# victordeleau/MUI-DeepAutoEncoder

Measured on NVIDIA B200. Metric: train samples/s, higher is better.
Workload: dtype bf16

## Files before the change

### include/codae_b200.h

```cpp
#ifndef CODAE_B200_H
#define CODAE_B200_H

#include <stddef.h>
#include <stdint.h>

#ifdef __cplusplus
extern "C" {
#endif

#define CODAE_VERSION 100

typedef struct codae_ctx codae_ctx;

enum codae_status { CODAE_OK = 0, CODAE_EINVAL = -1, CODAE_EARCH = -2, CODAE_ECUDA = -3, CODAE_ENOMEM = -4 };
enum codae_dtype { CODAE_F32 = 0, CODAE_BF16 = 1, CODAE_F32X3 = 2 };
enum codae_act { CODAE_ACT_NONE = 0, CODAE_ACT_RELU = 1 };
enum codae_metric { CODAE_METRIC_SQERR = 0, CODAE_METRIC_COSINE = 1 };
enum codae_vartype { CODAE_VAR_REGRESSION = 0, CODAE_VAR_CLASSIFICATION = 1 };
enum codae_engine { CODAE_ENGINE_SIMT_F32 = 0, CODAE_ENGINE_TCGEN05_BF16 = 1, CODAE_ENGINE_TCGEN05_F32X3 = 2 };

int codae_version(void);
int codae_ctx_create(int device, codae_ctx** out);
int codae_ctx_destroy(codae_ctx* ctx);
const char* codae_last_error(const codae_ctx* ctx);
int codae_ctx_sm_count(const codae_ctx* ctx);
enum codae_option { CODAE_OPT_SPLITK = 0, CODAE_OPT_PDL = 1, CODAE_OPT_PERSISTENT = 2, CODAE_OPT_WEIGHT_PREFETCH = 3,
                    CODAE_OPT_TMA_STORE = 4, CODAE_OPT_TMA_STORE_PERSISTENT = 5, CODAE_OPT_CTA_PAIR = 6 };
int codae_ctx_set_option(codae_ctx* ctx, int option, int value);
int codae_weights_written(codae_ctx* ctx, void* stream);
int codae_ctx_get_option(const codae_ctx* ctx, int option);
int codae_linear_engine(const codae_ctx* ctx, int dtype, int M, int N, int K);

int codae_mask_table_philox(codae_ctx* ctx, uint64_t seed, int64_t first_obs, int64_t n_obs, int nb_run,
                            int16_t* out, void* stream);

int codae_corrupt_fwd(codae_ctx* ctx, const float* data, int64_t n_rows, int64_t ld_data, const int64_t* batch_idx, int B,
                      const int16_t* mask_table, int nb_run, int run, const uint64_t* mask_bits,
                      const uint8_t* col_var, int io, void* out_cx, int cx_dtype, int64_t ld_cx, float* out_x,
                      int64_t ld_x, int32_t* out_mask_id, void* stream);

int codae_dense_masks(codae_ctx* ctx, const int64_t* batch_idx, int B, const int16_t* mask_table, int nb_run,
                      int run, const uint64_t* mask_bits, const uint8_t* nb_missing, const uint8_t* col_var, int io,
// ... 16 lines not shown
                        const float* norm_scale, const float* norm_min, int norm_first, const int32_t* mask_id,
                        const uint64_t* mask_bits, const uint8_t* nb_missing, int k_max, float* out_loss, double* acc,
                        void* stream);

int codae_linear_fwd(codae_ctx* ctx, const void* X, int64_t ldx, const void* W, int64_t ldw, const float* bias,
                     void* Y, int64_t ldy, int M, int N, int K, int act, int dtype, int out_dtype, void* stream);
int codae_linear_dgrad(codae_ctx* ctx, const void* dY, int64_t lddy, const void* W, int64_t ldw, const void* A_prev,
                       int64_t lda, void* dX, int64_t lddx, int M, int N, int K, int dtype, int out_dtype,
                       void* stream);
int codae_linear_wgrad(codae_ctx* ctx, const void* dY, int64_t lddy, const void* X, int64_t ldx, float* dW,
                       int64_t lddw, float* db, int M, int N, int K, int dtype, void* stream);
int codae_linear_wgrad_sq_slots(const codae_ctx* ctx, int M, int N, int K, int dtype);
int codae_linear_wgrad_sq(codae_ctx* ctx, const void* dY, int64_t lddy, const void* X, int64_t ldx, float* dW,
                          int64_t lddw, int M, int N, int K, int dtype, double* sq_partials, int n_slots,
                          void* stream);
int codae_linear_fwd_x3(codae_ctx* ctx, const void* X, int64_t ldx, int64_t x_plane, const void* W, int64_t ldw, int64_t w_plane,
                        void* Y, int64_t ldy, int64_t y_plane, int M, int N, int K, int act, int out_dtype, void* stream);
int codae_linear_dgrad_x3(codae_ctx* ctx, const void* dY, int64_t lddy, int64_t dy_plane, const void* W, int64_t ldw,
                          int64_t w_plane, const void* A_prev_hi, int64_t lda, void* dX, int64_t lddx, int64_t dx_plane, int M,
                          int N, int K, int out_dtype, void* stream);
int codae_linear_wgrad_x3(codae_ctx* ctx, const void* dY, int64_t lddy, int64_t dy_plane, const void* X, int64_t ldx,
                          int64_t x_plane, float* dW, int64_t lddw, int M, int N, int K, double* sq_partials, int n_slots,
                          void* stream);
int codae_split_x3(codae_ctx* ctx, const float* src, void* dst, int64_t n, int64_t plane_stride, void* stream);
typedef struct codae_tiny_layer {
    int64_t w_off;
    int32_t ld, bcol, in, out, relu;
} codae_tiny_layer;
int codae_tiny_mlp_fwd(codae_ctx* ctx, const codae_tiny_layer* layers, int n_layers, const float* flat, float* const* acts,
                       int64_t ld_act, int B, void* stream);
// ... 94 lines not shown
```

### mui-deepautoencoder_b200/codae/_C.py

```python
import ctypes
import os
import threading

import torch

_HERE = os.path.dirname(os.path.abspath(__file__))
LIB_PATH = os.path.join(_HERE, "_lib", "libcodae_b200.so")

OK, EINVAL, EARCH, ECUDA, ENOMEM = 0, -1, -2, -3, -4
F32, BF16, F32X3 = 0, 1, 2
ACT_NONE, ACT_RELU = 0, 1
METRIC_SQERR, METRIC_COSINE = 0, 1
VAR_REGRESSION, VAR_CLASSIFICATION = 0, 1
ENGINE_SIMT_F32, ENGINE_TCGEN05_BF16, ENGINE_TCGEN05_F32X3 = 0, 1, 2

_c = ctypes
_vp, _i, _i64, _u64, _f, _d, _sz = _c.c_void_p, _c.c_int, _c.c_int64, _c.c_uint64, _c.c_float, _c.c_double, _c.c_size_t

SIGNATURES = {
    "codae_version": (_i, []),
    "codae_ctx_create": (_i, [_i, _c.POINTER(_vp)]),
    "codae_ctx_destroy": (_i, [_vp]),
    "codae_last_error": (_c.c_char_p, [_vp]),
    "codae_ctx_sm_count": (_i, [_vp]),
# ... 2 lines not shown
    "codae_weights_written": (_i, [_vp, _vp]),
    "codae_linear_engine": (_i, [_vp, _i, _i, _i, _i]),
    "codae_mask_table_philox": (_i, [_vp, _u64, _i64, _i64, _i, _vp, _vp]),
    "codae_corrupt_fwd": (_i, [_vp, _vp, _i64, _i64, _vp, _i, _vp, _i, _i, _vp, _vp, _i, _vp, _i, _i64, _vp, _i64, _vp, _vp]),
    "codae_dense_masks": (_i, [_vp, _vp, _i, _vp, _i, _i, _vp, _vp, _vp, _i, _i, _vp, _vp, _vp]),
    "codae_mul_mask": (_i, [_vp, _vp, _vp, _vp, _i64, _vp]),
    "codae_loss_workspace_bytes": (_sz, [_vp]),
    "codae_mse_loss_fwd_bwd": (_i, [_vp, _vp, _i64, _vp, _vp, _i, _i64, _vp, _vp, _vp, _i, _i, _f, _vp, _i, _i64, _vp, _vp, _sz, _vp]),
    "codae_mixed_loss_fwd_bwd": (_i, [_vp, _vp, _vp, _i, _i, _i64, _i, _vp, _vp, _vp, _vp, _vp, _vp, _vp]),
    "codae_mixed_monitor": (_i, [_vp, _vp, _vp, _i, _i, _i64, _i, _vp, _vp, _vp, _vp, _vp, _i, _vp, _vp, _vp, _i, _vp, _vp, _vp]),
    "codae_linear_fwd": (_i, [_vp, _vp, _i64, _vp, _i64, _vp, _vp, _i64, _i, _i, _i, _i, _i, _i, _vp]),
    "codae_linear_dgrad": (_i, [_vp, _vp, _i64, _vp, _i64, _vp, _i64, _vp, _i64, _i, _i, _i, _i, _i, _vp]),
    "codae_linear_wgrad": (_i, [_vp, _vp, _i64, _vp, _i64, _vp, _i64, _vp, _i, _i, _i, _i, _vp]),
    "codae_linear_wgrad_sq_slots": (_i, [_vp, _i, _i, _i, _i]),
    "codae_linear_wgrad_sq": (_i, [_vp, _vp, _i64, _vp, _i64, _vp, _i64, _i, _i, _i, _i, _vp, _i, _vp]),
    "codae_linear_fwd_x3": (_i, [_vp, _vp, _i64, _i64, _vp, _i64, _i64, _vp, _i64, _i64, _i, _i, _i, _i, _i, _vp]),
    "codae_linear_dgrad_x3": (_i, [_vp, _vp, _i64, _i64, _vp, _i64, _i64, _vp, _i64, _vp, _i64, _i64, _i, _i, _i, _i, _vp]),
    "codae_linear_wgrad_x3": (_i, [_vp, _vp, _i64, _i64, _vp, _i64, _i64, _vp, _i64, _i, _i, _i, _vp, _i, _vp]),
    "codae_split_x3": (_i, [_vp, _vp, _vp, _i64, _i64, _vp]),
    "codae_tiny_mlp_fwd": (_i, [_vp, _vp, _i, _vp, _vp, _i64, _i, _vp]),
    "codae_tiny_mlp_bwd": (_i, [_vp, _vp, _i, _vp, _vp, _vp, _i64, _vp, _i64, _i, _vp]),
    "codae_cast_bf16": (_i, [_vp, _vp, _vp, _i64, _vp]),
    "codae_sqnorm_workspace_bytes": (_sz, [_vp]),
    "codae_grad_sqnorm": (_i, [_vp, _vp, _i64, _vp, _vp, _sz, _vp]),
    "codae_adam_step": (_i, [_vp, _vp, _vp, _vp, _vp, _vp, _i, _i64, _d, _d, _d, _d, _d, _i, _d, _vp, _d, _vp, _vp]),
    "codae_clip_adam_step": (_i, [_vp, _vp, _vp, _vp, _vp, _vp, _i, _i64, _d, _d, _d, _d, _d, _i, _d, _vp, _vp, _sz, _d, _vp, _vp]),
    "codae_adam_step_partials": (_i, [_vp, _vp, _vp, _vp, _vp, _vp, _i, _i64, _d, _d, _d, _d, _d, _i, _d, _vp, _i, _vp, _d, _vp, _vp]),
    "codae_counter_add": (_i, [_vp, _vp, _i, _vp]),
    "codae_dp_workspace_bytes": (_sz, [_vp]),
    "codae_dp_shard_elems": (_i64, [_i64, _i]),
# ... 74 lines not shown
    c = _ctxs.get(dev)
    if c is None:
        with _lock:
            c = _ctxs.get(dev)
            if c is None:
                out = _vp()
                rc = lib().codae_ctx_create(dev, ctypes.byref(out))
                if rc != OK:
                    raise RuntimeError("codae_ctx_create failed (%d): %s" % (rc, (lib().codae_last_error(None) or b"").decode()))
                c = out
                _ctxs[dev] = c
    return c


OPT_SPLITK, OPT_PDL, OPT_PERSISTENT, OPT_WEIGHT_PREFETCH, OPT_TMA_STORE, OPT_TMA_STORE_PERSISTENT, OPT_CTA_PAIR = 0, 1, 2, 3, 4, 5, 6


def set_option(device, option, value):
    c = ctx(device)
    check(lib().codae_ctx_set_option(c, option, 1 if value else 0), c)


def weights_written(device):
    c = ctx(device)
    check(lib().codae_weights_written(c, stream()), c)


def get_option(device, option):
    v = lib().codae_ctx_get_option(ctx(device), option)
    if v < 0:
# ... 147 lines not shown
def linear_wgrad(dY, X, dW, db, M, N, K, dtype):
    c = ctx(dY.device)
    if dtype == F32X3:
        assert is_x3(dY) and is_x3(X) and db is None, "codae: the fp32-parity engine takes the bias gradient from the augmented column"
        check(lib().codae_linear_wgrad_x3(c, p(dY), ld(dY), dY.stride(0), p(X), ld(X), X.stride(0), p(dW), dW.stride(0), M, N, K,
                                          None, 0, stream()), c)
        return
    check(lib().codae_linear_wgrad(c, p(dY), dY.stride(0), p(X), X.stride(0), p(dW), dW.stride(0), p(db), M, N, K, dtype,
                                   stream()), c)


def linear_wgrad_sq_slots(device, M, N, K, dtype):
    return int(lib().codae_linear_wgrad_sq_slots(ctx(device), M, N, K, dtype))


def linear_wgrad_sq(dY, X, dW, M, N, K, dtype, sq_partials):
    c = ctx(dY.device)
    if dtype == F32X3:
        assert is_x3(dY) and is_x3(X)
        check(lib().codae_linear_wgrad_x3(c, p(dY), ld(dY), dY.stride(0), p(X), ld(X), X.stride(0), p(dW), dW.stride(0), M, N, K,
                                          p(sq_partials), sq_partials.numel(), stream()), c)
        return
    check(lib().codae_linear_wgrad_sq(c, p(dY), dY.stride(0), p(X), X.stride(0), p(dW), dW.stride(0), M, N, K, dtype,
                                      p(sq_partials), sq_partials.numel(), stream()), c)


def split_x3(src, dst):
    assert dst.dtype == torch.bfloat16 and dst.shape[0] == 3 and src.dtype == torch.float32
    assert src.is_contiguous() and dst[0].is_contiguous() and dst[0].numel() == src.numel()
    c = ctx(src.device)
    check(lib().codae_split_x3(c, p(src), p(dst), src.numel(), dst.stride(0), stream()), c)
# ... 232 lines not shown
```

### mui-deepautoencoder_b200/codae/tool/fused_step.py

```python
import os

import torch

from codae import _C
from codae.tool.metering import arch_tables


def _round_up(x, m):
    return (x + m - 1) // m * m


class FusedStep:

    BUCKET_BYTES = 32 << 20

    def __init__(self, model, corrupter, data, lr, weight_decay, clip=True, betas=(0.9, 0.999), eps=1e-8,
                 max_norm=1.0, world_size=1, process_group=None, use_graph=False, mixed=None, overlap_allreduce=True,
                 fused_clip_adam=True, wgrad_sqnorm=None, tiny_mlp=None, dp_mode=None):
        if model.flat is None:
            raise RuntimeError("codae: FusedStep needs model.to(cuda_device) first; there is no CPU fallback")
        if not data.is_cuda:
            raise RuntimeError("codae: FusedStep needs dataset.to(cuda_device) first; there is no CPU fallback")
        self.model, self.corrupter, self.data = model, corrupter, data
        self.lr, self.wd, self.clip, self.betas, self.eps, self.max_norm = lr, weight_decay, clip, betas, eps, max_norm
        self.world_size, self.pg = world_size, process_group
        self.use_graph = use_graph
        self.mixed = mixed
        self.overlap_allreduce = overlap_allreduce
        self.fused_clip_adam = fused_clip_adam
# ... 139 lines not shown
        if self.adt == "x3":
            return _C.new_x3((B, w), self.dev)
        return torch.zeros((B, w), dtype=self.adt, device=self.dev)

    def _buffers(self, B):
        b = self._bufs.get(B)
        if b is None:
            dev, adt, dims = self.dev, self.adt, self.model.dims
            M = self.model
            wmax = max(M.act_width(max(i, o)) for i, o in dims)
            width = (lambda w: wmax) if self.mixed is not None else (lambda w: None)
            acts = [M.new_activation(B, dims[0][0], adt, dev, width(dims[0][0]))]
            for l, (i, o) in enumerate(dims):
                last = l == len(dims) - 1
                acts.append(M.new_activation(B, o, torch.float32 if last else adt, dev, width(o)))
            b = dict(acts=acts,
                     g0=self._new_grad(B, wmax), g1=self._new_grad(B, wmax), g2=self._new_grad(B, wmax),
                     mask_id=torch.zeros(B, dtype=torch.int32, device=dev),
                     idx=torch.zeros(B, dtype=torch.int64, device=dev),
                     x=torch.zeros((B, wmax), dtype=torch.float32, device=dev) if self.mixed is not None else None,
                     mon=torch.zeros((B, len(self.mixed["arch"])), dtype=torch.float32, device=dev) if self.mixed is not None else None)
            if self.wgrad_sqnorm:
                slots = [_C.linear_wgrad_sq_slots(dev, B, o, _round_up(i, 8) + 1, self.eng) for i, o in dims]
                if min(slots) < 1:
                    raise RuntimeError("codae: wgrad_sqnorm: the tensor-core engine cannot tile every layer of this model")
                offs = [0]
                for c in slots:
                    offs.append(offs[-1] + c)
                b["sq_off"] = offs
                b["sq_partials"] = torch.zeros(offs[-1], dtype=torch.float64, device=dev)
            self._bufs[B] = b
        return b

    def _enqueue(self, B, b, run, global_batch, data, idx, table, train=True):
        model, dims, eng = self.model, self.model.dims, self.eng
        L = len(dims)
        _, bits, col_var, nmiss = self.corrupter.device_tables()
        acts = b["acts"]
        n = 0
        _C.corrupt_fwd(data, idx, B, table, run, bits, col_var, self.io, acts[0], b["x"], b["mask_id"]); n += 1
        wflat = model.gemm_weights(eng)
        tiny = self.tiny_mlp and len({a.stride(0) for a in acts}) == 1
        if tiny:
            _C.tiny_mlp_fwd(self._tiny_layers, model.flat, acts, B); n += 1
        else:
            for l, (i, o) in enumerate(dims):
                _C.linear_fwd(acts[l], model.aug_view(wflat, l), None, acts[l + 1], B, o, _round_up(i, 8) + 1,
                              _C.ACT_RELU if model.relu[l] else _C.ACT_NONE, eng); n += 1
        y = acts[L]
        o_last = dims[L - 1][1]
        gbuf = [b["g0"], b["g1"], b["g2"]]
        g = gbuf[(L - 1) % 3][..., :_round_up(o_last, 8)]
        if self.mixed is None:
            _C.mse_loss_fwd_bwd(data, idx, y, b["mask_id"], bits, col_var, B, self.io, 2.0 / (global_batch * self.io),
                                g if train else None, self.acc, self.loss_ws); n += 1
        else:
            pos, size, typ = self.var_tables
            _C.mixed_loss_fwd_bwd(b["x"], y, pos, size, typ, self.weight, g, self.mixed_loss); n += 1
            _C.mixed_monitor(b["x"], y, pos, size, typ, self.norm_scale, self.norm_min, self.norm_first, b["mask_id"], bits,
                             nmiss, self.corrupter.k_max, b["mon"], self.mixed_acc); n += 1
        if not train:
            return n
        if tiny:
            _C.tiny_mlp_bwd(self._tiny_layers, model.flat, self.gflat, acts, gbuf, B); n += 1
            return n + self._enqueue_update(b.get("sq_partials"))
        overlap_comm = self.world_size > 1 and self.overlap_allreduce and self.dp_mode == "nccl"
        if overlap_comm:
            import torch.distributed as dist
        main = torch.cuda.current_stream()
        side = self._wgrad_stream if (self.tc and B <= 1024) else main
        wdone = [None] * L
        bucket_hi = None
        for l in range(L - 1, -1, -1):
            i, o = dims[l]
            gl = gbuf[l % 3][..., :_round_up(o, 8)]
            if side is not main:
                ready = torch.cuda.Event()
                ready.record(main)
                side.wait_event(ready)
            with torch.cuda.stream(side):
                if self.wgrad_sqnorm:
                    sq = b["sq_partials"][b["sq_off"][l]:b["sq_off"][l + 1]]
                    _C.linear_wgrad_sq(gl, acts[l], model.aug_view(self.gflat, l), B, o, _round_up(i, 8) + 1, eng, sq)
                else:
                    _C.linear_wgrad(gl, acts[l], model.aug_view(self.gflat, l), None, B, o, _round_up(i, 8) + 1, eng)
                n += 1
                wdone[l] = torch.cuda.Event()
                wdone[l].record(side)
            if overlap_comm:
                lo = self._layer_span[l][0]
                if bucket_hi is None:
                    bucket_hi = self._layer_span[l][1]
                if (bucket_hi - lo) * 4 >= self.BUCKET_BYTES or l == 0:
                    comm = self._comm_stream
                    comm.wait_event(wdone[l])
                    with torch.cuda.stream(comm):
                        dist.all_reduce(self.gflat[lo:bucket_hi], op=dist.ReduceOp.SUM, group=self.pg)
                    bucket_hi = None
            if l > 0:
                if l + 2 <= L - 1 and side is not main:
                    main.wait_event(wdone[l + 2])
                gp = gbuf[(l - 1) % 3][..., :_round_up(i, 8)]
                _C.linear_dgrad(gl, model.weight_view(wflat, l), acts[l] if model.relu[l - 1] else None, gp, B, o, i, eng); n += 1
        if side is not main:
            main.wait_stream(side)
        if overlap_comm:
            main.wait_stream(self._comm_stream)
        elif self.world_size > 1 and self.dp_mode == "nccl":
            import torch.distributed as dist
            dist.all_reduce(self.gflat, op=dist.ReduceOp.SUM, group=self.pg)
        return n + self._enqueue_update(b.get("sq_partials"))

    def _enqueue_update(self, sq_partials=None):
        model, eng = self.model, self.eng
        n = 0
        _C.counter_add(self.step_dev, 1); n += 1
        pb = model.gemm_weights(eng) if self.tc else None
# ... 183 lines not shown
```

### mui-deepautoencoder_b200/csrc/common.cuh

```cuda
#pragma once
#include <cuda_runtime.h>
#include <cuda_bf16.h>
#include <stdint.h>
#include <stdio.h>
#include <string.h>
#include <mutex>

#include "../../include/codae_b200.h"

struct CUtensorMap_st;

struct codae_ctx {
    int device;
    int sm_count;
    int cc_major, cc_minor;
    char err[512];
    void* encode_tiled;
    int splitk;
    int persistent;
    int pdl;
    int weight_prefetch;
    int tma_store;
    int tma_store_persistent;
    int cta_pair;
    int weights_dirty;
    cudaStream_t dirty_stream;
    std::mutex mu;
};

extern char g_codae_last_error[512];

int codae_fail(codae_ctx* ctx, int code, const char* fmt, ...);
int codae_check_launch(codae_ctx* ctx, const char* what);

#define CODAE_REQUIRE(ctx, cond, ...)                                     \
    do {                                                                  \
        if (!(cond)) return codae_fail((ctx), CODAE_EINVAL, __VA_ARGS__); \
    } while (0)

// ... 129 lines not shown
```

### mui-deepautoencoder_b200/csrc/ctx.cu

```cuda
#include <stdarg.h>
#include <stdlib.h>

#include "common.cuh"

char g_codae_last_error[512] = "";

int codae_fail(codae_ctx* ctx, int code, const char* fmt, ...) {
    char buf[512];
    va_list ap;
    va_start(ap, fmt);
    vsnprintf(buf, sizeof(buf), fmt, ap);
    va_end(ap);
    if (ctx) {
        std::lock_guard<std::mutex> lk(ctx->mu);
        snprintf(ctx->err, sizeof(ctx->err), "%s", buf);
    }
    snprintf(g_codae_last_error, sizeof(g_codae_last_error), "%s", buf);
    return code;
}

int codae_check_launch(codae_ctx* ctx, const char* what) {
    cudaError_t e = cudaPeekAtLastError();
    if (e != cudaSuccess) {
        cudaGetLastError();
// ... 48 lines not shown
    c->pdl = 1;
    c->persistent = 1;
    c->weight_prefetch = 1;
    {
        const char* e = getenv("CODAE_TMA_STORE");
        c->tma_store = e ? (atoi(e) != 0) : 1;
    }
    {
        const char* e = getenv("CODAE_TMA_STORE_PERSISTENT");
        c->tma_store_persistent = e ? (atoi(e) != 0) : 1;
    }
    {
        const char* e = getenv("CODAE_CTA_PAIR");
        c->cta_pair = e ? (atoi(e) != 0) : 1;
    }
    c->weights_dirty = 0;
    c->dirty_stream = nullptr;
    void* fn = nullptr;
    cudaDriverEntryPointQueryResult qres;
    e = cudaGetDriverEntryPoint("cuTensorMapEncodeTiled", &fn, cudaEnableDefault, &qres);
    if (e == cudaSuccess && qres == cudaDriverEntryPointSuccess) c->encode_tiled = fn;
    else cudaGetLastError();
    *out = c;
    return CODAE_OK;
}

int codae_ctx_destroy(codae_ctx* ctx) {
    delete ctx;
    return CODAE_OK;
}

const char* codae_last_error(const codae_ctx* ctx) { return ctx ? ctx->err : g_codae_last_error; }

int codae_ctx_sm_count(const codae_ctx* ctx) { return ctx ? ctx->sm_count : 0; }

int codae_ctx_set_option(codae_ctx* ctx, int option, int value) {
    if (!ctx) return codae_fail(nullptr, CODAE_EINVAL, "codae_ctx_set_option: ctx is NULL");
    if (option == CODAE_OPT_SPLITK) ctx->splitk = value ? 1 : 0;
    else if (option == CODAE_OPT_PDL) ctx->pdl = value ? 1 : 0;
    else if (option == CODAE_OPT_PERSISTENT) ctx->persistent = value ? 1 : 0;
    else if (option == CODAE_OPT_WEIGHT_PREFETCH) ctx->weight_prefetch = value ? 1 : 0;
    else if (option == CODAE_OPT_TMA_STORE) ctx->tma_store = value ? 1 : 0;
    else if (option == CODAE_OPT_TMA_STORE_PERSISTENT) ctx->tma_store_persistent = value ? 1 : 0;
    else if (option == CODAE_OPT_CTA_PAIR) ctx->cta_pair = value ? 1 : 0;
    else return codae_fail(ctx, CODAE_EINVAL, "codae_ctx_set_option: unknown option %d", option);
    return CODAE_OK;
}

int codae_weights_written(codae_ctx* ctx, void* stream) {
    if (!ctx) return codae_fail(nullptr, CODAE_EINVAL, "codae_weights_written: ctx is NULL");
    codae_mark_weights_written(ctx, as_stream(stream));
    return CODAE_OK;
}

int codae_ctx_get_option(const codae_ctx* ctx, int option) {
    if (!ctx) return CODAE_EINVAL;
    switch (option) {
        case CODAE_OPT_SPLITK: return ctx->splitk;
        case CODAE_OPT_PDL: return ctx->pdl;
        case CODAE_OPT_PERSISTENT: return ctx->persistent;
        case CODAE_OPT_WEIGHT_PREFETCH: return ctx->weight_prefetch;
        case CODAE_OPT_TMA_STORE: return ctx->tma_store;
        case CODAE_OPT_TMA_STORE_PERSISTENT: return ctx->tma_store_persistent;
        case CODAE_OPT_CTA_PAIR: return ctx->cta_pair;
        default: return CODAE_EINVAL;
    }
}

}
```

### mui-deepautoencoder_b200/csrc/gemm.h

```cpp
#pragma once
#include <cuda.h>

#include "common.cuh"

int codae_simt_linear_fwd(codae_ctx* ctx, const float* X, int64_t ldx, const float* W, int64_t ldw, const float* bias,
                          float* Y, int64_t ldy, int M, int N, int K, int act, cudaStream_t s);
int codae_simt_linear_dgrad(codae_ctx* ctx, const float* dY, int64_t lddy, const float* W, int64_t ldw, const float* A_prev,
                            int64_t lda, float* dX, int64_t lddx, int M, int N, int K, cudaStream_t s);
int codae_simt_linear_wgrad(codae_ctx* ctx, const float* dY, int64_t lddy, const float* X, int64_t ldx, float* dW,
                            int64_t lddw, int M, int N, int K, cudaStream_t s);
int codae_colsum(codae_ctx* ctx, const void* dY, int dtype, int64_t ld, int M, int N, float* db, cudaStream_t s);

struct Tc05Gemm {
    const void* A; int64_t lda; bool a_kmajor;
    const void* B; int64_t ldb; bool b_kmajor;
    void* C; int64_t ldc; int c_dtype;
    int M, N, K;
    const float* bias; int act;
    const void* mask_src; int64_t ldm;
    bool b_is_weight = false;
    double* sq_partial = nullptr;
    int sq_slots = 0;
    int planes = 1;
    int64_t a_plane_stride = 0, b_plane_stride = 0, c_plane_stride = 0;
};
bool codae_tc05_supported(const codae_ctx* ctx, const Tc05Gemm& g);
int codae_tc05_gemm(codae_ctx* ctx, const Tc05Gemm& g, cudaStream_t s);
int codae_tc05_gemm_ctas(const codae_ctx* ctx, const Tc05Gemm& g);
int codae_tc05_make_map(codae_ctx* ctx, CUtensorMap* map, const void* base, long long rows, long long cols, long long ld,
                        int box_cols, int box_rows, int planes, long long plane_stride);

struct ScoreTcPass {
    int metric;
    const void* cat; int cat_planes;
    int64_t cat_ld, cat_plane_stride;
    int64_t n_rows, row0;
    const __nv_bfloat16* q_planes;
    int64_t q_ld, q_plane_stride;
    int Q, E, qb0, G, W, kp;
    const float* cc;
    const float* qq;
    float inv_scale, c_rel;
    float* ls; int64_t* li;
// ... 5 lines not shown
```

### mui-deepautoencoder_b200/csrc/gemm_tcgen05.cu

```cuda
#include <cuda.h>
#include <stdlib.h>

#include "common.cuh"
#include "gemm.h"
#include "tc05_ptx.cuh"

namespace {

constexpr int kThreads = 192;
constexpr int kMaxSplit = 8;
inline int x3_chunk_kb() {
    static const int v = [] {
        const char* e = getenv("CODAE_X3_CHUNK_KB");
        const int x = e ? atoi(e) : 0;
        return x >= 1 && x <= 64 ? x : 8;
    }();
    return v;
}
constexpr uint32_t kPersistentStageBytes = 4 * 2 * 4096;

struct Params {
    int M, N, K;
    int a_kmajor, b_kmajor;
    void* C;
// ... 773 lines not shown
            if (lane == 0) asm volatile("cp.async.bulk.wait_group.read 0;" ::: "memory");
            __syncwarp();
        }
        if (p.sq_partial) sq_partial_store(p.sq_partial + blockIdx.x, sq_acc, sq_red);
    }
    tc_fence_before();
    if constexpr (kPair) cluster_sync();
    else __syncthreads();
    if (warp == 1) {
        tc_fence_after();
        if constexpr (kPair) tmem_dealloc_pair(tmem_base, 2 * BN);
        else tmem_dealloc(tmem_base, 2 * BN);
    }
}


int g_trace_cta = 0;
unsigned long long* g_trace_buf = nullptr;

typedef CUresult (*EncodeTiledFn)(CUtensorMap*, CUtensorMapDataType, cuuint32_t, void*, const cuuint64_t*, const cuuint64_t*,
                                  const cuuint32_t*, const cuuint32_t*, CUtensorMapInterleave, CUtensorMapSwizzle,
                                  CUtensorMapL2promotion, CUtensorMapFloatOOBfill);

int make_map(codae_ctx* ctx, CUtensorMap* map, const void* base, long long rows, long long cols, long long ld, int box_cols,
             int box_rows, int planes = 1, long long plane_stride = 0) {
    const cuuint64_t dims[3] = {(cuuint64_t)cols, (cuuint64_t)rows, (cuuint64_t)planes};
    const cuuint64_t strides[2] = {(cuuint64_t)ld * 2, (cuuint64_t)plane_stride * 2};
    const cuuint32_t box[3] = {(cuuint32_t)box_cols, (cuuint32_t)box_rows, 1};
    const cuuint32_t estr[3] = {1, 1, 1};
    CUresult r = reinterpret_cast<EncodeTiledFn>(ctx->encode_tiled)(
// ... 340 lines not shown
        case 256: return launch<256>(ctx, g, s);
        case 128: return launch<128>(ctx, g, s);
        default: return launch<64>(ctx, g, s);
    }
}

int codae_tc05_gemm_ctas(const codae_ctx* ctx, const Tc05Gemm& g) {
    if (!ctx || !ctx->encode_tiled || g.M < 1 || g.N < 32 || g.K < 1) return 0;
    if (g.planes == 3) return pick_bn(ctx, g) == 128 ? make_plan<128, 3>(ctx, g).ctas : make_plan<64, 3>(ctx, g).ctas;
    switch (pick_bn(ctx, g)) {
        case 256: return make_plan<256>(ctx, g).ctas;
        case 128: return make_plan<128>(ctx, g).ctas;
        default: return make_plan<64>(ctx, g).ctas;
    }
}
```

### mui-deepautoencoder_b200/csrc/linear.cu

```cuda
#include "common.cuh"
#include "gemm.h"

namespace {
inline bool tc_shape_ok(int M, int N, int K) { return M >= 1 && N >= 32 && K >= 32; }
}

extern "C" {

int codae_linear_engine(const codae_ctx* ctx, int dtype, int M, int N, int K) {
    if (!ctx) return CODAE_EINVAL;
    if (dtype == CODAE_BF16 && ctx->encode_tiled && tc_shape_ok(M, N, K))
        return CODAE_ENGINE_TCGEN05_BF16;
    if (dtype == CODAE_F32X3 && ctx->encode_tiled && tc_shape_ok(M, N, K)) return CODAE_ENGINE_TCGEN05_F32X3;
    return CODAE_ENGINE_SIMT_F32;
}

int codae_linear_fwd(codae_ctx* ctx, const void* X, int64_t ldx, const void* W, int64_t ldw, const float* bias, void* Y,
                     int64_t ldy, int M, int N, int K, int act, int dtype, int out_dtype, void* stream) {
    CODAE_REQUIRE(ctx, ctx && X && W && Y, "codae_linear_fwd: NULL argument");
    CODAE_REQUIRE(ctx, M >= 1 && N >= 1 && K >= 1 && ldx >= K && ldw >= K && ldy >= N, "codae_linear_fwd: bad shape M=%d N=%d K=%d", M, N, K);
    CODAE_REQUIRE(ctx, act == CODAE_ACT_NONE || act == CODAE_ACT_RELU, "codae_linear_fwd: bad activation %d", act);
    if (dtype == CODAE_F32) {
        CODAE_REQUIRE(ctx, out_dtype == CODAE_F32, "codae_linear_fwd: f32 engine writes f32");
        return codae_simt_linear_fwd(ctx, (const float*)X, ldx, (const float*)W, ldw, bias, (float*)Y, ldy, M, N, K, act, as_stream(stream));
// ... 41 lines not shown
    return codae_tc05_gemm_ctas(ctx, g);
}

int codae_linear_wgrad_sq(codae_ctx* ctx, const void* dY, int64_t lddy, const void* X, int64_t ldx, float* dW, int64_t lddw,
                          int M, int N, int K, int dtype, double* sq_partials, int n_slots, void* stream) {
    CODAE_REQUIRE(ctx, ctx && dY && X && dW && sq_partials, "codae_linear_wgrad_sq: NULL argument");
    CODAE_REQUIRE(ctx, M >= 1 && N >= 1 && K >= 1 && lddy >= N && ldx >= K && lddw >= K, "codae_linear_wgrad_sq: bad shape M=%d N=%d K=%d", M, N, K);
    CODAE_REQUIRE(ctx, dtype == CODAE_BF16, "codae_linear_wgrad_sq: tensor-core engine only (dtype %d)", dtype);
    CODAE_REQUIRE(ctx, (reinterpret_cast<uintptr_t>(sq_partials) & 7) == 0, "codae_linear_wgrad_sq: sq_partials must be 8-byte aligned");
    Tc05Gemm g{dY, lddy, false, X, ldx, false, dW, lddw, CODAE_F32, N, K, M, nullptr, CODAE_ACT_NONE, nullptr, 0};
    g.sq_partial = sq_partials;
    g.sq_slots = n_slots;
    return codae_tc05_gemm(ctx, g, as_stream(stream));
}

int codae_linear_fwd_x3(codae_ctx* ctx, const void* X, int64_t ldx, int64_t x_plane, const void* W, int64_t ldw, int64_t w_plane,
                        void* Y, int64_t ldy, int64_t y_plane, int M, int N, int K, int act, int out_dtype, void* stream) {
    CODAE_REQUIRE(ctx, ctx && X && W && Y, "codae_linear_fwd_x3: NULL argument");
    CODAE_REQUIRE(ctx, M >= 1 && N >= 1 && K >= 1 && ldx >= K && ldw >= K && ldy >= N, "codae_linear_fwd_x3: bad shape M=%d N=%d K=%d", M, N, K);
    CODAE_REQUIRE(ctx, act == CODAE_ACT_NONE || act == CODAE_ACT_RELU, "codae_linear_fwd_x3: bad activation %d", act);
    CODAE_REQUIRE(ctx, out_dtype == CODAE_F32 || out_dtype == CODAE_F32X3, "codae_linear_fwd_x3: output is f32 or its bf16 triple");
    Tc05Gemm g{X, ldx, true, W, ldw, true, Y, ldy, out_dtype, M, N, K, nullptr, act, nullptr, 0, true};
    g.planes = 3; g.a_plane_stride = x_plane; g.b_plane_stride = w_plane; g.c_plane_stride = y_plane;
    return codae_tc05_gemm(ctx, g, as_stream(stream));
}

int codae_linear_dgrad_x3(codae_ctx* ctx, const void* dY, int64_t lddy, int64_t dy_plane, const void* W, int64_t ldw,
                          int64_t w_plane, const void* A_prev_hi, int64_t lda, void* dX, int64_t lddx, int64_t dx_plane, int M,
                          int N, int K, int out_dtype, void* stream) {
    CODAE_REQUIRE(ctx, ctx && dY && W && dX, "codae_linear_dgrad_x3: NULL argument");
// ... 22 lines not shown
```

Measured before the change: 1.244 million.

## Batch all layers' weight-gradient GEMMs into one grouped persistent tcgen05 launch

Adds a grouped persistent CTA-pair kernel that computes the weight gradients of every layer in a single launch, using a segment table to map tile items to problems. The backward pass first runs every dgrad, then issues this one grouped wgrad call instead of interleaving per-layer wgrad launches on a side stream. The aim is to cut launch overhead and fill the tail of small per-layer GEMMs by load-balancing tiles across all SMs. In exchange, wgrad can no longer overlap with dgrad, one gradient buffer per layer is needed instead of three, and the path only applies to large bf16 batches when sqnorm or peer mode is enabled.

After: 1.275 million (median of 6 runs). 2.5% higher.

```diff
diff --git a/include/codae_b200.h b/include/codae_b200.h
--- a/include/codae_b200.h
+++ b/include/codae_b200.h
@@ -25,7 +25,8 @@
 const char* codae_last_error(const codae_ctx* ctx);
 int codae_ctx_sm_count(const codae_ctx* ctx);
 enum codae_option { CODAE_OPT_SPLITK = 0, CODAE_OPT_PDL = 1, CODAE_OPT_PERSISTENT = 2, CODAE_OPT_WEIGHT_PREFETCH = 3,
-                    CODAE_OPT_TMA_STORE = 4, CODAE_OPT_TMA_STORE_PERSISTENT = 5, CODAE_OPT_CTA_PAIR = 6 };
+                    CODAE_OPT_TMA_STORE = 4, CODAE_OPT_TMA_STORE_PERSISTENT = 5, CODAE_OPT_CTA_PAIR = 6,
+                    CODAE_OPT_GROUPED_WGRAD = 7 };
 int codae_ctx_set_option(codae_ctx* ctx, int option, int value);
 int codae_weights_written(codae_ctx* ctx, void* stream);
 int codae_ctx_get_option(const codae_ctx* ctx, int option);
@@ -72,6 +73,10 @@
 int codae_linear_wgrad_sq(codae_ctx* ctx, const void* dY, int64_t lddy, const void* X, int64_t ldx, float* dW,
                           int64_t lddw, int M, int N, int K, int dtype, double* sq_partials, int n_slots,
                           void* stream);
+int codae_linear_wgrad_sq_grouped_slots(const codae_ctx* ctx, int n, const int* M, const int* N, const int* K, int dtype);
+int codae_linear_wgrad_sq_grouped(codae_ctx* ctx, int n, const void* const* dY, const int64_t* lddy, const void* const* X,
+                                  const int64_t* ldx, float* const* dW, const int64_t* lddw, const int* M, const int* N,
+                                  const int* K, int dtype, double* sq_partials, int n_slots, void* stream);
 int codae_linear_fwd_x3(codae_ctx* ctx, const void* X, int64_t ldx, int64_t x_plane, const void* W, int64_t ldw, int64_t w_plane,
                         void* Y, int64_t ldy, int64_t y_plane, int M, int N, int K, int act, int out_dtype, void* stream);
 int codae_linear_dgrad_x3(codae_ctx* ctx, const void* dY, int64_t lddy, int64_t dy_plane, const void* W, int64_t ldw,
diff --git a/mui-deepautoencoder_b200/codae/_C.py b/mui-deepautoencoder_b200/codae/_C.py
--- a/mui-deepautoencoder_b200/codae/_C.py
+++ b/mui-deepautoencoder_b200/codae/_C.py
@@ -40,6 +40,8 @@
     "codae_linear_wgrad": (_i, [_vp, _vp, _i64, _vp, _i64, _vp, _i64, _vp, _i, _i, _i, _i, _vp]),
     "codae_linear_wgrad_sq_slots": (_i, [_vp, _i, _i, _i, _i]),
     "codae_linear_wgrad_sq": (_i, [_vp, _vp, _i64, _vp, _i64, _vp, _i64, _i, _i, _i, _i, _vp, _i, _vp]),
+    "codae_linear_wgrad_sq_grouped_slots": (_i, [_vp, _i, _vp, _vp, _vp, _i]),
+    "codae_linear_wgrad_sq_grouped": (_i, [_vp, _i, _vp, _vp, _vp, _vp, _vp, _vp, _vp, _vp, _vp, _i, _vp, _i, _vp]),
     "codae_linear_fwd_x3": (_i, [_vp, _vp, _i64, _i64, _vp, _i64, _i64, _vp, _i64, _i64, _i, _i, _i, _i, _i, _vp]),
     "codae_linear_dgrad_x3": (_i, [_vp, _vp, _i64, _i64, _vp, _i64, _i64, _vp, _i64, _vp, _i64, _i64, _i, _i, _i, _i, _vp]),
     "codae_linear_wgrad_x3": (_i, [_vp, _vp, _i64, _i64, _vp, _i64, _i64, _vp, _i64, _i, _i, _i, _vp, _i, _vp]),
@@ -144,6 +146,7 @@
 
 
 OPT_SPLITK, OPT_PDL, OPT_PERSISTENT, OPT_WEIGHT_PREFETCH, OPT_TMA_STORE, OPT_TMA_STORE_PERSISTENT, OPT_CTA_PAIR = 0, 1, 2, 3, 4, 5, 6
+OPT_GROUPED_WGRAD = 7
 
 
 def set_option(device, option, value):
@@ -321,7 +324,26 @@
     return int(lib().codae_linear_wgrad_sq_slots(ctx(device), M, N, K, dtype))
 
 
+def _arr(ctype, vals):
+    return (ctype * len(vals))(*vals)
+
+
+def linear_wgrad_sq_grouped_slots(device, M, N, K, dtype):
+    n = len(M)
+    return int(lib().codae_linear_wgrad_sq_grouped_slots(ctx(device), n, _arr(_i, M), _arr(_i, N), _arr(_i, K), dtype))
+
+
 def linear_wgrad_sq(dY, X, dW, M, N, K, dtype, sq_partials):
+    if isinstance(dY, (list, tuple)):
+        c = ctx(dY[0].device)
+        n = len(dY)
+        assert len(X) == len(dW) == len(M) == len(N) == len(K) == n
+        check(lib().codae_linear_wgrad_sq_grouped(c, n, _arr(_vp, [t.data_ptr() for t in dY]), _arr(_i64, [t.stride(0) for t in dY]),
+                                                  _arr(_vp, [t.data_ptr() for t in X]), _arr(_i64, [t.stride(0) for t in X]),
+                                                  _arr(_vp, [t.data_ptr() for t in dW]), _arr(_i64, [t.stride(0) for t in dW]),
+                                                  _arr(_i, M), _arr(_i, N), _arr(_i, K), dtype, p(sq_partials),
+                                                  0 if sq_partials is None else sq_partials.numel(), stream()), c)
+        return
     c = ctx(dY.device)
     if dtype == F32X3:
         assert is_x3(dY) and is_x3(X)
diff --git a/mui-deepautoencoder_b200/codae/tool/fused_step.py b/mui-deepautoencoder_b200/codae/tool/fused_step.py
--- a/mui-deepautoencoder_b200/codae/tool/fused_step.py
+++ b/mui-deepautoencoder_b200/codae/tool/fused_step.py
@@ -13,6 +13,7 @@
 class FusedStep:
 
     BUCKET_BYTES = 32 << 20
+    SMALL_BATCH = 1024
 
     def __init__(self, model, corrupter, data, lr, weight_decay, clip=True, betas=(0.9, 0.999), eps=1e-8,
                  max_norm=1.0, world_size=1, process_group=None, use_graph=False, mixed=None, overlap_allreduce=True,
@@ -182,13 +183,15 @@
             for l, (i, o) in enumerate(dims):
                 last = l == len(dims) - 1
                 acts.append(M.new_activation(B, o, torch.float32 if last else adt, dev, width(o)))
-            b = dict(acts=acts,
-                     g0=self._new_grad(B, wmax), g1=self._new_grad(B, wmax), g2=self._new_grad(B, wmax),
+            grouped = self._grouped_wgrad_slots(B)
+            b = dict(acts=acts, gbuf=[self._new_grad(B, wmax) for _ in range(len(dims) if grouped else 3)], grouped=grouped > 0,
                      mask_id=torch.zeros(B, dtype=torch.int32, device=dev),
                      idx=torch.zeros(B, dtype=torch.int64, device=dev),
                      x=torch.zeros((B, wmax), dtype=torch.float32, device=dev) if self.mixed is not None else None,
                      mon=torch.zeros((B, len(self.mixed["arch"])), dtype=torch.float32, device=dev) if self.mixed is not None else None)
-            if self.wgrad_sqnorm:
+            if self.wgrad_sqnorm and grouped:
+                b["sq_partials"] = torch.zeros(grouped, dtype=torch.float64, device=dev)
+            elif self.wgrad_sqnorm:
                 slots = [_C.linear_wgrad_sq_slots(dev, B, o, _round_up(i, 8) + 1, self.eng) for i, o in dims]
                 if min(slots) < 1:
                     raise RuntimeError("codae: wgrad_sqnorm: the tensor-core engine cannot tile every layer of this model")
@@ -199,6 +202,13 @@
                 b["sq_partials"] = torch.zeros(offs[-1], dtype=torch.float64, device=dev)
             self._bufs[B] = b
         return b
+
+    def _grouped_wgrad_slots(self, B):
+        if self.eng != _C.BF16 or B <= self.SMALL_BATCH or not (self.wgrad_sqnorm or self.dp_mode == "peer"):
+            return 0
+        dims = self.model.dims
+        return _C.linear_wgrad_sq_grouped_slots(self.dev, [B] * len(dims), [o for _, o in dims],
+                                                [_round_up(i, 8) + 1 for i, _ in dims], self.eng)
 
     def _enqueue(self, B, b, run, global_batch, data, idx, table, train=True):
         model, dims, eng = self.model, self.model.dims, self.eng
@@ -217,8 +227,8 @@
                               _C.ACT_RELU if model.relu[l] else _C.ACT_NONE, eng); n += 1
         y = acts[L]
         o_last = dims[L - 1][1]
-        gbuf = [b["g0"], b["g1"], b["g2"]]
-        g = gbuf[(L - 1) % 3][..., :_round_up(o_last, 8)]
+        gbuf = b["gbuf"]
+        g = gbuf[(L - 1) % len(gbuf)][..., :_round_up(o_last, 8)]
         if self.mixed is None:
             _C.mse_loss_fwd_bwd(data, idx, y, b["mask_id"], bits, col_var, B, self.io, 2.0 / (global_batch * self.io),
                                 g if train else None, self.acc, self.loss_ws); n += 1
@@ -232,16 +242,25 @@
         if tiny:
             _C.tiny_mlp_bwd(self._tiny_layers, model.flat, self.gflat, acts, gbuf, B); n += 1
             return n + self._enqueue_update(b.get("sq_partials"))
+        if b["grouped"]:
+            for l in range(L - 1, 0, -1):
+                i, o = dims[l]
+                _C.linear_dgrad(gbuf[l][..., :_round_up(o, 8)], model.weight_view(wflat, l), acts[l] if model.relu[l - 1] else None,
+                                gbuf[l - 1][..., :_round_up(i, 8)], B, o, i, eng); n += 1
+            _C.linear_wgrad_sq([gbuf[l][..., :_round_up(o, 8)] for l, (i, o) in enumerate(dims)], acts[:L],
+                               [model.aug_view(self.gflat, l) for l in range(L)], [B] * L, [o for _, o in dims],
+                               [_round_up(i, 8) + 1 for i, _ in dims], eng, b.get("sq_partials")); n += 1
+            return n + self._enqueue_update(b.get("sq_partials"))
         overlap_comm = self.world_size > 1 and self.overlap_allreduce and self.dp_mode == "nccl"
         if overlap_comm:
             import torch.distributed as dist
         main = torch.cuda.current_stream()
-        side = self._wgrad_stream if (self.tc and B <= 1024) else main
+        side = self._wgrad_stream if (self.tc and B <= self.SMALL_BATCH) else main
         wdone = [None] * L
         bucket_hi = None
         for l in range(L - 1, -1, -1):
             i, o = dims[l]
-            gl = gbuf[l % 3][..., :_round_up(o, 8)]
+            gl = gbuf[l % len(gbuf)][..., :_round_up(o, 8)]
             if side is not main:
                 ready = torch.cuda.Event()
                 ready.record(main)
@@ -268,7 +287,7 @@
             if l > 0:
                 if l + 2 <= L - 1 and side is not main:
                     main.wait_event(wdone[l + 2])
-                gp = gbuf[(l - 1) % 3][..., :_round_up(i, 8)]
+                gp = gbuf[(l - 1) % len(gbuf)][..., :_round_up(i, 8)]
                 _C.linear_dgrad(gl, model.weight_view(wflat, l), acts[l] if model.relu[l - 1] else None, gp, B, o, i, eng); n += 1
         if side is not main:
             main.wait_stream(side)
diff --git a/mui-deepautoencoder_b200/csrc/common.cuh b/mui-deepautoencoder_b200/csrc/common.cuh
--- a/mui-deepautoencoder_b200/csrc/common.cuh
+++ b/mui-deepautoencoder_b200/csrc/common.cuh
@@ -23,6 +23,7 @@
     int tma_store;
     int tma_store_persistent;
     int cta_pair;
+    int grouped_wgrad;
     int weights_dirty;
     cudaStream_t dirty_stream;
     std::mutex mu;
diff --git a/mui-deepautoencoder_b200/csrc/ctx.cu b/mui-deepautoencoder_b200/csrc/ctx.cu
--- a/mui-deepautoencoder_b200/csrc/ctx.cu
+++ b/mui-deepautoencoder_b200/csrc/ctx.cu
@@ -86,6 +86,10 @@
         const char* e = getenv("CODAE_CTA_PAIR");
         c->cta_pair = e ? (atoi(e) != 0) : 1;
     }
+    {
+        const char* e = getenv("CODAE_GROUPED_WGRAD");
+        c->grouped_wgrad = e ? (atoi(e) != 0) : 1;
+    }
     c->weights_dirty = 0;
     c->dirty_stream = nullptr;
     void* fn = nullptr;
@@ -115,6 +119,7 @@
     else if (option == CODAE_OPT_TMA_STORE) ctx->tma_store = value ? 1 : 0;
     else if (option == CODAE_OPT_TMA_STORE_PERSISTENT) ctx->tma_store_persistent = value ? 1 : 0;
     else if (option == CODAE_OPT_CTA_PAIR) ctx->cta_pair = value ? 1 : 0;
+    else if (option == CODAE_OPT_GROUPED_WGRAD) ctx->grouped_wgrad = value ? 1 : 0;
     else return codae_fail(ctx, CODAE_EINVAL, "codae_ctx_set_option: unknown option %d", option);
     return CODAE_OK;
 }
@@ -135,6 +140,7 @@
         case CODAE_OPT_TMA_STORE: return ctx->tma_store;
         case CODAE_OPT_TMA_STORE_PERSISTENT: return ctx->tma_store_persistent;
         case CODAE_OPT_CTA_PAIR: return ctx->cta_pair;
+        case CODAE_OPT_GROUPED_WGRAD: return ctx->grouped_wgrad;
         default: return CODAE_EINVAL;
     }
 }
diff --git a/mui-deepautoencoder_b200/csrc/gemm.h b/mui-deepautoencoder_b200/csrc/gemm.h
--- a/mui-deepautoencoder_b200/csrc/gemm.h
+++ b/mui-deepautoencoder_b200/csrc/gemm.h
@@ -27,6 +27,8 @@
 bool codae_tc05_supported(const codae_ctx* ctx, const Tc05Gemm& g);
 int codae_tc05_gemm(codae_ctx* ctx, const Tc05Gemm& g, cudaStream_t s);
 int codae_tc05_gemm_ctas(const codae_ctx* ctx, const Tc05Gemm& g);
+int codae_tc05_wgrad_grouped_ctas(const codae_ctx* ctx, int n, const Tc05Gemm* gs);
+int codae_tc05_wgrad_grouped(codae_ctx* ctx, int n, const Tc05Gemm* gs, double* sq_partial, int sq_slots, cudaStream_t s);
 int codae_tc05_make_map(codae_ctx* ctx, CUtensorMap* map, const void* base, long long rows, long long cols, long long ld,
                         int box_cols, int box_rows, int planes, long long plane_stride);
 
diff --git a/mui-deepautoencoder_b200/csrc/gemm_tcgen05.cu b/mui-deepautoencoder_b200/csrc/gemm_tcgen05.cu
--- a/mui-deepautoencoder_b200/csrc/gemm_tcgen05.cu
+++ b/mui-deepautoencoder_b200/csrc/gemm_tcgen05.cu
@@ -811,6 +811,189 @@
     }
 }
 
+constexpr int kMaxGroup = 16;
+struct GroupedProblem {
+    float* C;
+    long long ldc;
+    int M, N, num_kb;
+};
+struct GroupedSegment {
+    int first, prob, tiles_m, tiles_n, n_idx0;
+};
+struct GroupedArgs {
+    CUtensorMap a[kMaxGroup], b[kMaxGroup], c[kMaxGroup];
+    GroupedProblem pr[kMaxGroup];
+    GroupedSegment seg[2 * kMaxGroup];
+    int n_seg, n_items, group_m;
+    double* sq_partial;
+};
+
+__device__ __forceinline__ void grouped_item(const GroupedArgs& g, int t, int& prob, int& m_idx, int& n_idx) {
+    int s = 0;
+    while (s + 1 < g.n_seg && t >= g.seg[s + 1].first) ++s;
+    prob = g.seg[s].prob;
+    tile_coords(t - g.seg[s].first, g.seg[s].tiles_m, g.seg[s].tiles_n, g.group_m, m_idx, n_idx);
+    n_idx += g.seg[s].n_idx0;
+}
+
+__global__ void __launch_bounds__(kThreads, 1) tc05_wgrad_grouped_kernel(const __grid_constant__ GroupedArgs g) {
+    constexpr int BN = 256;
+    using C = PCfg<BN, true>;
+    constexpr int kRowsPerTile = 2 * BM;
+    extern __shared__ uint8_t smem_raw[];
+    uint8_t* smem = reinterpret_cast<uint8_t*>((reinterpret_cast<uintptr_t>(smem_raw) + 1023) & ~uintptr_t(1023));
+    constexpr int kS = C::kStages;
+    uint8_t* stage_base = smem + kS * C::kStageBytes;
+    uint64_t* full_bar = reinterpret_cast<uint64_t*>(stage_base + kPersistentStageBytes);
+    uint64_t* empty_bar = full_bar + kS;
+    uint64_t* tmem_full_bar = empty_bar + kS;
+    uint64_t* tmem_empty_bar = tmem_full_bar + 2;
+    uint32_t* tmem_slot = reinterpret_cast<uint32_t*>(tmem_empty_bar + 2);
+    __shared__ double sq_red[4];
+
+    pdl_launch_dependents();
+    const int warp = threadIdx.x >> 5, lane = threadIdx.x & 31;
+    const int rank = (int)cluster_ctarank();
+    const int worker = (int)(blockIdx.x >> 1), num_workers = (int)(gridDim.x >> 1);
+
+    if (warp == 0 && lane == 0) {
+        for (int s = 0; s < kS; ++s) { mbar_init(&full_bar[s], 1); mbar_init(&empty_bar[s], 1); }
+        for (int a = 0; a < 2; ++a) { mbar_init(&tmem_full_bar[a], 1); mbar_init(&tmem_empty_bar[a], 8); }
+        asm volatile("fence.mbarrier_init.release.cluster;" ::: "memory");
+        asm volatile("fence.proxy.async.shared::cta;" ::: "memory");
+    }
+    if (warp == 1) tmem_alloc_pair(tmem_slot, 2 * BN);
+    tc_fence_before();
+    cluster_sync();
+    tc_fence_after();
+    const uint32_t tmem_base = *tmem_slot;
+    pdl_wait();
+
+    if (warp == 0) {
+        if (lane == 0) {
+            int s = 0;
+            uint32_t ph = 0;
+            for (int t = worker; t < g.n_items; t += num_workers) {
+                int pi, m_idx, n_idx;
+                grouped_item(g, t, pi, m_idx, n_idx);
+                const int N = g.pr[pi].N, num_kb = g.pr[pi].num_kb;
+                const CUtensorMap* ma = &g.a[pi];
+                const CUtensorMap* mb = &g.b[pi];
+                const int m0 = m_idx * kRowsPerTile + rank * BM, n0 = n_idx * BN;
+                const int n_half = min(BN, ((N - n0) + 31) & ~31) >> 1;
+                const int nb0 = n0 + rank * n_half;
+                for (int kb = 0; kb < num_kb; ++kb, s = (s + 1 == kS ? 0 : s + 1), ph ^= (s == 0)) {
+                    mbar_wait(&empty_bar[s], ph ^ 1);
+                    uint8_t* a_dst = smem + s * C::kStageBytes;
+                    uint8_t* b_dst = a_dst + kATileBytes;
+                    if (rank == 0) mbar_expect_tx(&full_bar[s], 2 * C::kStageBytes);
+                    const uint32_t bar = mapa_u32(smem_u32(&full_bar[s]), 0);
+                    const int k0 = kb * BK;
+                    tma_load_2d_pair(ma, bar, a_dst, m0, k0);
+                    tma_load_2d_pair(ma, bar, a_dst + 8192, m0 + 64, k0);
+                    tma_load_2d_pair(mb, bar, b_dst, nb0, k0);
+                    tma_load_2d_pair(mb, bar, b_dst + 8192, nb0 + 64, k0);
+                }
+            }
+        }
+    } else if (warp == 1) {
+        if (lane == 0 && rank == 0) {
+            constexpr uint32_t adv = UMMA_K * 128;
+            int s = 0;
+            uint32_t ph = 0;
+            int it = 0;
+            for (int t = worker; t < g.n_items; t += num_workers, ++it) {
+                int pi, m_idx, n_idx;
+                grouped_item(g, t, pi, m_idx, n_idx);
+                const int num_kb = g.pr[pi].num_kb;
+                const int n_eff = min(BN, ((g.pr[pi].N - n_idx * BN) + 31) & ~31);
+                const uint32_t idesc = make_idesc(n_eff, false, false, kRowsPerTile);
+                const int acc = it & 1;
+                const uint32_t acc_ph = (it >> 1) & 1;
+                mbar_wait_cluster(&tmem_empty_bar[acc], acc_ph ^ 1);
+                tc_fence_after();
+                const uint32_t d_tmem = tmem_base + (uint32_t)(acc * BN);
+                for (int kb = 0; kb < num_kb; ++kb, s = (s + 1 == kS ? 0 : s + 1), ph ^= (s == 0)) {
+                    mbar_wait(&full_bar[s], ph);
+                    tc_fence_after();
+                    const uint32_t a_addr = smem_u32(smem + s * C::kStageBytes);
+                    const uint32_t b_addr = a_addr + kATileBytes;
+#pragma unroll
+                    for (int k = 0; k < BK / UMMA_K; ++k)
+                        umma_bf16_pair(d_tmem, make_desc(a_addr + k * adv, false), make_desc(b_addr + k * adv, false), idesc,
+                                       (kb | k) != 0);
+                    umma_commit_pair(&empty_bar[s]);
+                }
+                umma_commit_pair(&tmem_full_bar[acc]);
+            }
+        }
+    } else {
+        const int q = warp & 3;
+        int it = 0;
+        double sq_acc = 0.0;
+        uint8_t* wbuf = stage_base + q * 8192;
+        int unit = 0;
+        for (int t = worker; t < g.n_items; t += num_workers, ++it) {
+            const int acc = it & 1;
+            const uint32_t acc_ph = (it >> 1) & 1;
+            int pi, m_idx, n_idx;
+            grouped_item(g, t, pi, m_idx, n_idx);
+            const int M = g.pr[pi].M, N = g.pr[pi].N, n4 = N & ~3;
+            const int m0 = m_idx * kRowsPerTile + rank * BM, n0 = n_idx * BN;
+            mbar_wait(&tmem_full_bar[acc], acc_ph);
+            tc_fence_after();
+            const int row = m0 + q * 32 + lane;
+            const bool row_ok = row < M;
+            const int n_chunks = min(BN / 32, (N - n0 + 31) / 32);
+#pragma unroll 1
+            for (int c = 0; c < n_chunks; ++c) {
+                uint32_t v[32];
+                tmem_ld32(tmem_base + ((uint32_t)(q * 32) << 16) + (uint32_t)(acc * BN + c * 32), v);
+                if (c == n_chunks - 1) {
+                    tc_fence_before();
+                    __syncwarp();
+                    if (lane == 0) mbar_arrive_cluster(mapa_u32(smem_u32(&tmem_empty_bar[acc]), 0));
+                }
+                const int col0 = n0 + c * 32;
+                float f[32];
+#pragma unroll
+                for (int j = 0; j < 32; ++j) f[j] = __uint_as_float(v[j]);
+                if (row_ok && g.sq_partial) sq_acc += (double)chunk_sq<32>(f, col0, N);
+                uint8_t* box = wbuf + (unit & 1) * 4096;
+                if (lane == 0) asm volatile("cp.async.bulk.wait_group.read 1;" ::: "memory");
+                __syncwarp();
+                uint8_t* brow = box + lane * 128;
+                const int sw = lane & 7;
+#pragma unroll
+                for (int j = 0; j < 8; ++j)
+                    *reinterpret_cast<float4*>(brow + ((j ^ sw) << 4)) = make_float4(f[4 * j], f[4 * j + 1], f[4 * j + 2], f[4 * j + 3]);
+                if (row_ok && n4 < N && n4 >= col0 && n4 < col0 + 32) {
+                    float* crow = g.pr[pi].C + (long long)row * g.pr[pi].ldc;
+#pragma unroll
+                    for (int j = 0; j < 32; ++j)
+                        if (col0 + j >= n4 && col0 + j < N) crow[col0 + j] = f[j];
+                }
+                asm volatile("fence.proxy.async.shared::cta;" ::: "memory");
+                __syncwarp();
+                if (lane == 0) {
+                    if (col0 < n4 && m0 + q * 32 < M) tma_store_2d(&g.c[pi], box, col0, m0 + q * 32);
+                    asm volatile("cp.async.bulk.commit_group;" ::: "memory");
+                }
+                ++unit;
+            }
+        }
+        if (lane == 0) asm volatile("cp.async.bulk.wait_group.read 0;" ::: "memory");
+        __syncwarp();
+        if (g.sq_partial) sq_partial_store(g.sq_partial + blockIdx.x, sq_acc, sq_red);
+    }
+    tc_fence_before();
+    cluster_sync();
+    if (warp == 1) {
+        tc_fence_after();
+        tmem_dealloc_pair(tmem_base, 2 * BN);
+    }
+}
+
 
 int g_trace_cta = 0;
 unsigned long long* g_trace_buf = nullptr;
@@ -1181,3 +1364,110 @@
         default: return make_plan<64>(ctx, g).ctas;
     }
 }
+
+static bool grouped_problem_ok(const codae_ctx* ctx, const Tc05Gemm& g) {
+    if (!codae_tc05_supported(ctx, g) || g.planes != 1 || g.a_kmajor || g.b_kmajor || g.c_dtype != CODAE_F32 || g.bias ||
+        g.act != CODAE_ACT_NONE || g.mask_src)
+        return false;
+    return pick_bn(ctx, g) == 256 && make_plan<256>(ctx, g).pair;
+}
+
+int codae_tc05_wgrad_grouped_ctas(const codae_ctx* ctx, int n, const Tc05Gemm* gs) {
+    if (!ctx || !ctx->grouped_wgrad || n < 1) return 0;
+    for (int i = 0; i < n; ++i)
+        if (!grouped_problem_ok(ctx, gs[i])) return 0;
+    return ((n + kMaxGroup - 1) / kMaxGroup) * (ctx->sm_count & ~1);
+}
+
+int codae_tc05_wgrad_grouped(codae_ctx* ctx, int n, const Tc05Gemm* gs, double* sq_partial, int sq_slots, cudaStream_t s) {
+    const int slots = codae_tc05_wgrad_grouped_ctas(ctx, n, gs);
+    if (slots == 0)
+        return codae_fail(ctx, CODAE_EINVAL, "codae_tc05_wgrad_grouped: not a grouped plan (option off, or a problem that would not "
+                          "run as a persistent CTA-pair launch on its own, or an unsupported shape / alignment)");
+    if (sq_partial && sq_slots != slots)
+        return codae_fail(ctx, CODAE_EINVAL, "codae_tc05_wgrad_grouped: %d sum-of-squares slots passed, these launches write %d",
+                          sq_slots, slots);
+    using PC = PCfg<256, true>;
+    const unsigned smem = PC::kSmemBytes + kPersistentStageBytes;
+    static bool attr_set = false;
+    if (!attr_set) {
+        cudaError_t e = cudaFuncSetAttribute(tc05_wgrad_grouped_kernel, cudaFuncAttributeMaxDynamicSharedMemorySize, (int)smem);
+        if (e != cudaSuccess) return codae_fail(ctx, CODAE_ECUDA, "cudaFuncSetAttribute(smem=%u): %s", smem, cudaGetErrorString(e));
+        attr_set = true;
+    }
+    static const int env_group_m = [] {
+        const char* e = getenv("CODAE_GROUP_M");
+        return (e && atoi(e) > 0) ? atoi(e) : 16;
+    }();
+    const int ctas = ctx->sm_count & ~1;
+    for (int c0 = 0; c0 < n; c0 += kMaxGroup) {
+        const int cn = n - c0 < kMaxGroup ? n - c0 : kMaxGroup;
+        GroupedArgs ga;
+        memset(&ga, 0, sizeof(ga));
+        int item = 0, nseg = 0;
+        for (int i = 0; i < cn; ++i) {
+            const Tc05Gemm& g = gs[c0 + i];
+            int rc = make_map(ctx, &ga.a[i], g.A, g.K, g.M, g.lda, 64, BK);
+            if (!rc) rc = make_map(ctx, &ga.b[i], g.B, g.K, g.N, g.ldb, 64, BK);
+            if (!rc) rc = make_store_map(ctx, &ga.c[i], g.C, CODAE_F32, g.M, g.N & ~3, g.ldc, 32);
+            if (rc) return rc;
+            ga.pr[i].C = static_cast<float*>(g.C);
+            ga.pr[i].ldc = g.ldc;
+            ga.pr[i].M = g.M;
+            ga.pr[i].N = g.N;
+            ga.pr[i].num_kb = (g.K + BK - 1) / BK;
+            const int tiles_m = (g.M + 2 * BM - 1) / (2 * BM), full_n = g.N / 256;
+            if (full_n > 0) {
+                ga.seg[nseg++] = GroupedSegment{item, i, tiles_m, full_n, 0};
+                item += tiles_m * full_n;
+            }
+        }
+        int order[kMaxGroup], nn = 0;
+        for (int i = 0; i < cn; ++i)
+            if (gs[c0 + i].N % 256) order[nn++] = i;
+        auto width = [&](int i) { return ((gs[c0 + i].N % 256) + 31) & ~31; };
+        for (int a = 1; a < nn; ++a)
+            for (int b = a; b > 0 && width(order[b]) > width(order[b - 1]); --b) {
+                const int t = order[b]; order[b] = order[b - 1]; order[b - 1] = t;
+            }
+        for (int j = 0; j < nn; ++j) {
+            const Tc05Gemm& g = gs[c0 + order[j]];
+            const int tiles_m = (g.M + 2 * BM - 1) / (2 * BM);
+            ga.seg[nseg++] = GroupedSegment{item, order[j], tiles_m, 1, g.N / 256};
+            item += tiles_m;
+        }
+        ga.n_seg = nseg;
+        ga.n_items = item;
+        ga.group_m = env_group_m > 1 ? env_group_m / 2 : 1;
+        ga.sq_partial = sq_partial ? sq_partial + (size_t)(c0 / kMaxGroup) * ctas : nullptr;
+        cudaLaunchConfig_t cfg = {};
+        cfg.gridDim = dim3(ctas);
+        cfg.blockDim = dim3(kThreads);
+        cfg.dynamicSmemBytes = smem;
+        cfg.stream = s;
+        cudaLaunchAttribute attr[2];
+        attr[0].id = cudaLaunchAttributeClusterDimension;
+        attr[0].val.clusterDim.x = 2;
+        attr[0].val.clusterDim.y = 1;
+        attr[0].val.clusterDim.z = 1;
+        int na = 1;
+        if (codae_pdl_allowed(ctx, s)) {
+            attr[na].id = cudaLaunchAttributeProgrammaticStreamSerialization;
+            attr[na].val.programmaticStreamSerializationAllowed = 1;
+            ++na;
+        }
+        cfg.attrs = attr;
+        cfg.numAttrs = na;
+        static const bool debug_plan = getenv("CODAE_DEBUG_PLAN") != nullptr;
+        if (debug_plan)
+            fprintf(stderr, "codae plan: grouped wgrad, %d problems, %d segments, %d items, ctas %d\n", cn, nseg, item, ctas);
+        cudaError_t le = cudaLaunchKernelEx(&cfg, tc05_wgrad_grouped_kernel, ga);
+        if (le != cudaSuccess) {
+            cudaGetLastError();
+            return codae_fail(ctx, CODAE_ECUDA, "tc05_wgrad_grouped_kernel launch: %s", cudaGetErrorString(le));
+        }
+        const int rc = codae_check_launch(ctx, "tc05_wgrad_grouped_kernel");
+        if (rc) return rc;
+    }
+    return CODAE_OK;
+}
diff --git a/mui-deepautoencoder_b200/csrc/linear.cu b/mui-deepautoencoder_b200/csrc/linear.cu
--- a/mui-deepautoencoder_b200/csrc/linear.cu
+++ b/mui-deepautoencoder_b200/csrc/linear.cu
@@ -1,5 +1,7 @@
 #include "common.cuh"
 #include "gemm.h"
+
+#include <vector>
 
 namespace {
 inline bool tc_shape_ok(int M, int N, int K) { return M >= 1 && N >= 32 && K >= 32; }
@@ -79,6 +81,35 @@
     return codae_tc05_gemm(ctx, g, as_stream(stream));
 }
 
+int codae_linear_wgrad_sq_grouped_slots(const codae_ctx* ctx, int n, const int* M, const int* N, const int* K, int dtype) {
+    if (!ctx || dtype != CODAE_BF16 || n < 1 || !M || !N || !K) return 0;
+    std::vector<Tc05Gemm> gs;
+    for (int i = 0; i < n; ++i) {
+        if (!tc_shape_ok(M[i], N[i], K[i])) return 0;
+        gs.push_back(Tc05Gemm{nullptr, 0, false, nullptr, 0, false, nullptr, 0, CODAE_F32, N[i], K[i], M[i], nullptr, CODAE_ACT_NONE,
+                              nullptr, 0});
+    }
+    return codae_tc05_wgrad_grouped_ctas(ctx, n, gs.data());
+}
+
+int codae_linear_wgrad_sq_grouped(codae_ctx* ctx, int n, const void* const* dY, const int64_t* lddy, const void* const* X,
+                                  const int64_t* ldx, float* const* dW, const int64_t* lddw, const int* M, const int* N,
+                                  const int* K, int dtype, double* sq_partials, int n_slots, void* stream) {
+    CODAE_REQUIRE(ctx, ctx && n >= 1 && dY && lddy && X && ldx && dW && lddw && M && N && K,
+                  "codae_linear_wgrad_sq_grouped: NULL argument or n < 1");
+    CODAE_REQUIRE(ctx, dtype == CODAE_BF16, "codae_linear_wgrad_sq_grouped: bf16 tensor-core engine only (dtype %d)", dtype);
+    CODAE_REQUIRE(ctx, (reinterpret_cast<uintptr_t>(sq_partials) & 7) == 0, "codae_linear_wgrad_sq_grouped: sq_partials must be 8-byte aligned");
+    std::vector<Tc05Gemm> gs;
+    for (int i = 0; i < n; ++i) {
+        CODAE_REQUIRE(ctx, dY[i] && X[i] && dW[i], "codae_linear_wgrad_sq_grouped: NULL operand of layer %d", i);
+        CODAE_REQUIRE(ctx, M[i] >= 1 && N[i] >= 1 && K[i] >= 1 && lddy[i] >= N[i] && ldx[i] >= K[i] && lddw[i] >= K[i],
+                      "codae_linear_wgrad_sq_grouped: bad shape of layer %d: M=%d N=%d K=%d", i, M[i], N[i], K[i]);
+        gs.push_back(Tc05Gemm{dY[i], lddy[i], false, X[i], ldx[i], false, dW[i], lddw[i], CODAE_F32, N[i], K[i], M[i], nullptr,
+                              CODAE_ACT_NONE, nullptr, 0});
+    }
+    return codae_tc05_wgrad_grouped(ctx, n, gs.data(), sq_partials, n_slots, as_stream(stream));
+}
+
 int codae_linear_fwd_x3(codae_ctx* ctx, const void* X, int64_t ldx, int64_t x_plane, const void* W, int64_t ldw, int64_t w_plane,
                         void* Y, int64_t ldy, int64_t y_plane, int M, int N, int K, int act, int out_dtype, void* stream) {
     CODAE_REQUIRE(ctx, ctx && X && W && Y, "codae_linear_fwd_x3: NULL argument");
```
